# jl6017/AutoURDF

Measured on AMD Instinct MI355X. Metric: registered frames/sec (N=4096 pts, K=20 clusters), higher is better.
Workload: dtype f32

## Files before the change

### autourdf_amd/_lib.py

```python
import ctypes
import os

import torch

_HERE = os.path.dirname(os.path.abspath(__file__))
_VARIANT = os.environ.get("CREG_LIB_VARIANT", "")
LIB_PATH = os.path.join(_HERE, "libcreg" + ("_" + _VARIANT if _VARIANT else "") + ".so")

vp, i64, i32, f32, f64, sz = (ctypes.c_void_p, ctypes.c_int64, ctypes.c_int32, ctypes.c_float,
                              ctypes.c_double, ctypes.c_size_t)


class TrainShape(ctypes.Structure):
    _fields_ = [("rot", i32), ("k", i32), ("hidden", i32), ("epochs", i32), ("n_pred", i64),
                ("n_tgt", i64), ("use_graph", i32), ("batch", i32), ("graph_branches", i32), ("nn_search", i32)]


class TrainArgs(ctypes.Structure):
    _fields_ = [("m", vp), ("y", vp), ("local_pts", vp), ("seg_offsets", vp),
                ("params", ctypes.POINTER(vp)), ("lr", f32), ("sched_factor", f32),
                ("sched_patience", i32), ("stop", i32), ("best_m", vp), ("best_pred", vp),
                ("loss_hist", vp), ("lr_hist", vp), ("result", vp), ("y_unchanged", i32), ("reserved_", i32)]


# ... 56 lines not shown
    "creg_depth_points_f64": (ctypes.c_int, [vp, vp, i32, f64, f64, i32, i32, vp, sz, vp, i64, vp]),
    "creg_segment_plane_workspace_bytes": (sz, [i64, i32, i32]),
    "creg_segment_plane_f64": (ctypes.c_int, [vp, i64, vp, i32, vp, i32, i32, f64, vp, vp, vp, vp, vp, vp, vp, sz, vp]),
    "creg_mesh_collide_workspace_bytes": (sz, [i64, i32, i64, i64]),
    "creg_mesh_collide_f64": (ctypes.c_int, [vp, vp, i64, vp, i32, i64, vp, i64, vp, vp, vp, vp, sz, vp]),
    "creg_urdf_fk_f64": (ctypes.c_int, [vp, vp, vp, vp, vp, i32, i32, i32, vp, i32, vp, vp, vp, vp]),
    "creg_coord_dist_map_workspace_bytes": (sz, [i32, i32]),
    "creg_coord_dist_map_f64": (ctypes.c_int, [vp, i32, i32, f64, i32, vp, vp, vp, sz, vp]),
    "creg_pose_coords_f64": (ctypes.c_int, [vp, i64, vp, vp]),
    "creg_link_sweep_f64": (ctypes.c_int, [vp, i32, i32, i32, vp, vp, vp, vp, vp, vp]),
    "creg_coord_mst_f64": (ctypes.c_int, [vp, i32, i32, vp, vp, vp]),
    "creg_joint_axes_samples": (ctypes.c_int, [i32, i32, i32]),
    "creg_joint_axes_f64": (ctypes.c_int, [vp, i32, i32, i32, vp, vp, i32, vp, i32, i32, i32, i32, vp, vp, vp, vp, vp, vp, vp,
                                           vp, vp, vp, vp]),
    "creg_link_clouds_f64": (ctypes.c_int, [vp, vp, i32, i32, vp, vp, i32, i32, vp, vp, i64, vp, i64, i64, vp, vp, vp, vp,
                                            vp]),
    "creg_statistical_outlier_f64": (ctypes.c_int, [vp, i64, vp, i32, i32, f64, vp, vp, vp, vp]),
    "creg_voxel_bounds_f64": (ctypes.c_int, [vp, i64, vp, i32, vp, f64, vp, vp, vp, vp]),
    "creg_voxel_layout": (ctypes.c_int, [vp, vp, i32, vp]),
    "creg_voxel_fill_f64": (ctypes.c_int, [vp, i64, vp, i32, vp, f64, vp, vp, vp, i64, vp, vp]),
    "creg_mc_workspace_bytes": (sz, [i64]),
    "creg_mc_count_u8": (ctypes.c_int, [vp, vp, vp, i32, i64, vp, vp, vp, sz, vp]),
    "creg_mc_emit_i32": (ctypes.c_int, [vp, vp, i32, i64, vp, i64, i64, vp, vp, vp, sz, vp]),
    "creg_mesh_finish_workspace_bytes": (sz, [i64]),
    "creg_mesh_finish_f64": (ctypes.c_int, [vp, i64, vp, i64, vp, vp, i32, vp, f64, i32, vp, vp, vp, sz, vp]),
    "creg_train_workspace_bytes": (sz, [ctypes.POINTER(TrainShape)]),
    "creg_train_plan_create": (ctypes.c_int, [ctypes.POINTER(TrainShape), vp, sz, ctypes.POINTER(vp)]),
    "creg_train_plan_run": (ctypes.c_int, [vp, ctypes.POINTER(TrainArgs), vp]),
    "creg_train_plan_run_batch": (ctypes.c_int, [vp, ctypes.POINTER(TrainArgs), i32, vp]),
    "creg_train_plan_resume": (ctypes.c_int, [vp, ctypes.POINTER(TrainArgs), ctypes.POINTER(TrainState), i32, ctypes.POINTER(vp), ctypes.POINTER(vp), vp, vp]),
    "creg_train_plan_probe": (ctypes.c_int, [vp, ctypes.POINTER(TrainArgs), vp, vp, vp, vp, vp]),
    "creg_train_plan_profile": (ctypes.c_int, [vp, ctypes.POINTER(TrainArgs), i32, ctypes.POINTER(f32), vp]),
    "creg_train_plan_info": (ctypes.c_int, [vp, vp]),
    "creg_train_plan_destroy": (ctypes.c_int, [vp]),
}

_lib = None


def load(check_device: bool = True) -> ctypes.CDLL:
    global _lib
    if _lib is None:
        if not os.path.exists(LIB_PATH):
            raise RuntimeError(
                f"{LIB_PATH} is missing: build it with `python -m autourdf_amd.build` "
                "(hipcc --offload-arch=gfx950). autourdf_amd has no CPU fallback.")
        hip = os.path.join(os.path.dirname(torch.__file__), "lib", "libamdhip64.so")
        if os.path.exists(hip):
            ctypes.CDLL(hip, mode=ctypes.RTLD_GLOBAL)
        L = ctypes.CDLL(LIB_PATH)
        for name, (res, args) in SIGNATURES.items():
            fn = getattr(L, name)
            fn.restype, fn.argtypes = res, args
        _lib = L
    if check_device:
        rc = _lib.creg_device_check()
        if rc != 0:
            raise RuntimeError("libcreg needs an MI355X (gfx950): " + _lib.creg_last_error().decode())
    return _lib


def check(rc: int, what: str = "libcreg call"):
    if rc != 0:
        raise RuntimeError(f"{what} failed ({rc}): {_lib.creg_last_error().decode()}")


# ... 8 lines not shown
```

### autourdf_amd/csrc/train_engine.hip

```cpp
#include <cfloat>
#include <chrono>
#include <cmath>
#include <cstdlib>
#include <cstring>
#include <type_traits>
#include <vector>
#include "creg_common.h"
#include "nn_l1.h"

namespace creg {

struct Dims {
    int rot, K, KP, IN, H, HA, HB, H2, OA, OB, NP, NT, epochs;
    float slope;
    int oW1, ob1, oW2, ob2, oW3A, ob3A, oW3B, ob3B, NPAR;
    int nbx, nby;
    int nyb;
    int npb;
    int ppl;
    int nbt, nbp;
    int rows;
};

constexpr int PS_MAXB = 512;
// ... 1 lines not shown
struct Hyper {
    float lr, factor;
    int patience, stop;
};

struct TrainState {
    double lr, sched_best;
    int sched_bad, count, stopped, step;
    float min_loss;
    int epochs_run, best_epoch;
    float step_size, bc2_sqrt;
    float last_loss;
    float next_bc2s;
    double next_bc1;
};

struct Ws {
    float *P, *P1, *AM, *AV;
    float *pose_in, *enc, *x1[2], *h2[2], *head_save, *m2, *gm2;
    float4 *pts4, *y4, *pred4, *ys4, *psl4, *ps4;
    float *ybox, *pbox;
    int* sb;
    int* sgn_x;
    int4* cnt4;
    float *lossp_x, *lossp_y;
    float *g_out, *g_h2;
    TrainState* state;
    double* bc1;
    float* bc2s;
    float *best_m, *best_pred, *loss_hist, *lr_hist, *result;
    int* off;
    Hyper* hyper;
    unsigned long long* ysum;
};

static_assert(sizeof(Ws) % sizeof(char*) == 0, "Ws must hold pointers only");
__host__ __device__ __forceinline__ Ws ws_shift(Ws W, size_t bytes) {
    char** p = reinterpret_cast<char**>(&W);
#pragma unroll
    for (size_t i = 0; i < sizeof(Ws) / sizeof(char*); ++i) p[i] += bytes;
    return W;
}

constexpr int ROT_Q = 0, ROT_DQ = 1, ROT_6D = 2, ROT_RPY = 3;
constexpr int POSE_IN = 12;
__device__ __forceinline__ float act_f(float v, float slope) { return v > 0.f ? v : v * slope; }
__device__ __forceinline__ float act_grad(float post, float slope) { return post > 0.f ? 1.f : slope; }

__device__ __forceinline__ int seg_of(const int* __restrict__ off, int k, int n) {
    int lo = 0, hi = k;
    while (hi - lo > 1) { const int mid = (lo + hi) >> 1; if (off[mid] <= n) lo = mid; else hi = mid; }
    return lo;
}

constexpr int PREP_MAXB = 64;
struct PrepBatch { const float* m[PREP_MAXB]; const float* y[PREP_MAXB]; const float* pts[PREP_MAXB]; Hyper hy[PREP_MAXB]; };
__global__ __launch_bounds__(256) void k_prep(Dims D, Ws W0, size_t bstride, PrepBatch pb) {
    const Ws W = ws_shift(W0, blockIdx.z * bstride);
    const Hyper hy = pb.hy[blockIdx.z];
    const float* __restrict__ m = pb.m[blockIdx.z];
    const float* __restrict__ y = pb.y[blockIdx.z];
    const float* __restrict__ pts = pb.pts[blockIdx.z];
    const int t = blockIdx.x * 256 + threadIdx.x;
    const int stride = gridDim.x * 256;
    for (int n = t; n < D.NP; n += stride) {
        const int c = seg_of(W.off, D.K, n);
// ... 71 lines not shown
}

typedef float f32x4 __attribute__((ext_vector_type(4)));
constexpr int L2_THREADS = 512;
constexpr int L2_RB = 32;
template <int NC>
__device__ __forceinline__ void l2_body(const Dims& D, const Ws& W, int par, int blk) {
    constexpr int KW = 8 * NC, NS = KW / 4;
    constexpr bool V4 = KW % 16 == 0;
    constexpr int NL = V4 ? NS / 4 : NS;
    __shared__ __attribute__((aligned(16))) float red[(L2_THREADS / 64) * L2_RB * 16];
    const float* Pc = par ? W.P1 : W.P;
    const float* x1cur = par ? W.x1[1] : W.x1[0];
    float* h2out = par ? W.h2[1] : W.h2[0];
    const int tid = threadIdx.x, lane = tid & 63, wv = tid >> 6, lj = lane & 15, kk = lane >> 4;
    const int u0 = blk * 16, H = D.H;
    auto load_t = [&](const float* rowp, float* dst) {
        const float* p = rowp + wv * KW + (V4 ? 4 * kk : kk);
#pragma unroll
        for (int q = 0; q < NL; ++q) {
            if constexpr (V4) { const float4 v = *(const float4*)(p + 16 * q); dst[4 * q] = v.x; dst[4 * q + 1] = v.y; dst[4 * q + 2] = v.z; dst[4 * q + 3] = v.w; }
            else dst[q] = p[4 * q];
        }
    };
    float bw[NS], a0[NS], a1[NS];
    load_t(Pc + D.oW2 + (size_t)(u0 + lj) * H, bw);
    load_t(x1cur + (size_t)min(lj, D.K - 1) * H, a0);
    const bool two0 = D.K > 16;
    if (two0) load_t(x1cur + (size_t)min(16 + lj, D.K - 1) * H, a1);
    const float bias = Pc[D.ob2 + u0 + (tid & 15)];
    __builtin_amdgcn_sched_barrier(0);
    const int stopped = W.state[par].stopped;
    __builtin_amdgcn_sched_barrier(0);
    for (int r0 = 0; r0 < D.K; r0 += L2_RB) {
        const int nr = min(L2_RB, D.K - r0);
        const bool two = nr > 16;
        if (r0) {
            load_t(x1cur + (size_t)min(r0 + lj, D.K - 1) * H, a0);
            if (two) load_t(x1cur + (size_t)min(r0 + 16 + lj, D.K - 1) * H, a1);
        }
        f32x4 acc0 = {0.f, 0.f, 0.f, 0.f}, acc1 = {0.f, 0.f, 0.f, 0.f};
        if (two) {
#pragma unroll
            for (int s = 0; s < NS; ++s) {
                acc0 = __builtin_amdgcn_mfma_f32_16x16x4f32(a0[s], bw[s], acc0, 0, 0, 0);
                acc1 = __builtin_amdgcn_mfma_f32_16x16x4f32(a1[s], bw[s], acc1, 0, 0, 0);
            }
        } else {
#pragma unroll
            for (int s = 0; s < NS; ++s) acc0 = __builtin_amdgcn_mfma_f32_16x16x4f32(a0[s], bw[s], acc0, 0, 0, 0);
        }
        if (r0) __syncthreads();
        {
            float* o = red + (wv * L2_RB + 4 * kk) * 16 + lj;
#pragma unroll
            for (int v = 0; v < 4; ++v) { o[v * 16] = acc0[v]; if (two) o[(16 + v) * 16] = acc1[v]; }
        }
        __syncthreads();
        if (stopped) return;
        if (tid < nr * 16) {
            float sum = red[tid];
#pragma unroll
            for (int w2 = 1; w2 < L2_THREADS / 64; ++w2) sum += red[w2 * L2_RB * 16 + tid];
            h2out[(size_t)(r0 + (tid >> 4)) * D.H2 + u0 + (tid & 15)] = act_f(sum + bias, D.slope);
        }
    }
}
template <int NC>
__global__ __launch_bounds__(L2_THREADS) void k_l2(Dims D, Ws W0, int par, size_t bstride) {
    asm volatile("" :: "s"(W0.P), "s"(W0.P1), "s"(W0.x1[0]), "s"(W0.x1[1]), "s"(W0.h2[0]), "s"(W0.h2[1]), "s"(W0.state), "s"(D.K), "s"(D.H),
                 "s"(D.H2), "s"(D.oW2), "s"(D.ob2), "s"(D.slope), "s"(par), "s"(bstride));
    const Ws W = ws_shift(W0, blockIdx.z * bstride);
    l2_body<NC>(D, W, par, blockIdx.x);
}

template <int NC, bool X = false>
__global__ __launch_bounds__(512) void k_head(Dims D, Ws W0, int par, size_t bstride) {
    asm volatile("" :: "s"(W0.P), "s"(W0.P1), "s"(W0.h2[0]), "s"(W0.h2[1]), "s"(W0.pose_in), "s"(W0.head_save), "s"(W0.m2), "s"(W0.pts4), "s"(W0.pred4),
                 "s"(W0.psl4), "s"(W0.ps4), "s"(W0.pbox), "s"(W0.sb), "s"(W0.cnt4), "s"(W0.state), "s"(W0.off), "s"(D.rot), "s"(D.K), "s"(D.H2), "s"(D.HA),
                 "s"(D.HB), "s"(D.OA), "s"(D.OB), "s"(D.NP), "s"(D.npb), "s"(D.ppl), "s"(D.nbp), "s"(D.oW3A), "s"(D.ob3A), "s"(D.oW3B), "s"(D.ob3B), "s"(par),
                 "s"(bstride));
    const Ws W = ws_shift(W0, blockIdx.z * bstride);
    const float* h2cur = par ? W.h2[1] : W.h2[0];
    const float* Pc = par ? W.P1 : W.P;
    __shared__ float outs[12];
    __shared__ float m2s[12];
    const int r = blockIdx.x, lane = threadIdx.x & 63, wave = threadIdx.x >> 6;
    const int NO = D.OA + D.OB;
    const int o = min(wave, (X ? 8 : NO) - 1);
    const float *w, *a; int n;
    if (o < D.OA) { w = Pc + D.oW3A + (size_t)o * D.HA; a = h2cur + (size_t)r * D.H2; n = D.HA; }
    else { w = Pc + D.oW3B + (size_t)(o - D.OA) * D.HB; a = h2cur + (size_t)r * D.H2 + D.HA; n = D.HB; }
    float wv[NC], av[NC];
#pragma unroll
    for (int c = 0; c < NC; ++c) { const int i = min(c * 64 + lane, n - 1); wv[c] = w[i]; av[c] = a[i]; }
    const float bias = o < D.OA ? Pc[D.ob3A + o] : Pc[D.ob3B + o - D.OA];
    float wv9[NC], av9[NC], bias9 = 0.f;
    if constexpr (X) {
        const float* w9 = Pc + D.oW3B + (size_t)(8 - D.OA) * D.HB;
        const float* a9 = h2cur + (size_t)r * D.H2 + D.HA;
#pragma unroll
        for (int c = 0; c < NC; ++c) { const int i = min(c * 64 + lane, D.HB - 1); wv9[c] = w9[i]; av9[c] = a9[i]; }
        bias9 = Pc[D.ob3B + 8 - D.OA];
// ... 594 lines not shown
constexpr int B2_WAVES = B2_THREADS / 64;
constexpr int B2_CB = 16;
constexpr int B2_RB = 32;
__host__ __device__ inline int b2_smem_floats(int K, int IN, int H2) {
    return B2_WAVES * B2_RB * B2_CB + K * IN + 2 * K * B2_CB + H2 * B2_CB;
}
__device__ __forceinline__ float row_sum16(float v) {
    CREG_DPP_STEP(v, 0xB1, 0xF);
    CREG_DPP_STEP(v, 0x4E, 0xF);
    CREG_DPP_STEP(v, 0x141, 0xF);
    CREG_DPP_STEP(v, 0x140, 0xF);
    return v;
}

template <int KW, bool X>
__device__ __forceinline__ void bwd2_role(const Dims& D, const Ws& W, int epoch, int blk, float* sh, unsigned long long bd_entry) {
    constexpr int NS = KW / 4;
    constexpr bool V4 = KW % 16 == 0;
    constexpr int NA = V4 ? NS / 4 : NS;
    float* red = sh;
    float* encs = red + B2_WAVES * B2_RB * B2_CB;
    float* gxs = encs + D.K * D.IN;
    float* xt = gxs + D.K * B2_CB;
    float* w2s = xt + D.K * B2_CB;
    const int tid = threadIdx.x, lane = tid & 63, wv = tid >> 6, lj = lane & 15, kk = lane >> 4;
    __builtin_amdgcn_s_waitcnt(0x0F70);
    const int c0 = blk * B2_CB, par = epoch & 1;
    const float* x1cur = par ? W.x1[1] : W.x1[0];
    float* x1next = par ? W.x1[0] : W.x1[1];
    const float* Pc = par ? W.P1 : W.P;
    float* Pn = par ? W.P : W.P1;
    BD_T0
    {
        const float* src = Pc + D.oW2 + (size_t)(wv * KW + (lane >> 2)) * D.H + c0 + 4 * (lane & 3);
        float* dst = w2s + wv * KW * B2_CB;
#pragma unroll
        for (int i = 0; i < KW; i += 16)
            if (i + (lane >> 2) < KW)
                __builtin_amdgcn_global_load_lds((const __attribute__((address_space(1))) void*)(src + (size_t)i * D.H),
                                                 (__attribute__((address_space(3))) void*)(dst + i * B2_CB), 16, 0, 0);
    }
    const float* gbase = W.g_h2 + wv * KW + (V4 ? 4 * kk : kk);
    auto load_a = [&](int row, float* dst) {
        const float* g = gbase + (size_t)min(row, D.K - 1) * D.H2;
#pragma unroll
        for (int q = 0; q < NA; ++q) {
            if constexpr (V4) { const float4 v = *(const float4*)(g + 16 * q); dst[4 * q] = v.x; dst[4 * q + 1] = v.y; dst[4 * q + 2] = v.z; dst[4 * q + 3] = v.w; }
            else dst[q] = g[4 * q];
        }
    };
    float a0[NS], a1[NS];
    const bool two0 = D.K > 16;
    load_a(lj, a0);
    if (two0) load_a(16 + lj, a1);
    const int half = tid >> 8, t2 = tid & 255, row = t2 >> 4, i4 = t2 & 15, hu = c0 + row;
    const bool ain = 4 * i4 < D.IN;
    const int ei = min(4 * i4, D.IN - 4);
    const size_t wi = (size_t)D.oW1 + (size_t)hu * D.IN + ei;
    float4 pw = *(const float4*)(Pc + wi), pm = *(const float4*)(W.AM + wi), pv = *(const float4*)(W.AV + wi);
    const bool ain2 = X && 64 + 4 * i4 < D.IN;
    const int ei2 = min(64 + 4 * i4, D.IN - 4);
    const size_t wi2 = (size_t)D.oW1 + (size_t)hu * D.IN + ei2;
    float4 pw2, pm2, pv2;
    if constexpr (X) { pw2 = *(const float4*)(Pc + wi2); pm2 = *(const float4*)(W.AM + wi2); pv2 = *(const float4*)(W.AV + wi2); }
    float pb = Pc[D.ob1 + hu], mb = W.AM[D.ob1 + hu], vb = W.AV[D.ob1 + hu];
    float xv0 = x1cur[(size_t)min(tid >> 4, D.K - 1) * D.H + c0 + (tid & 15)];
    {
        const int n = D.K * D.IN / 4;
        constexpr int NPC = 8;
#pragma unroll
        for (int c = 0; c < NPC; ++c) {
            const int i = c * B2_THREADS + tid;
// ... 181 lines not shown
        mfma_ops();
    }
    BD_T
    if (S.stopped) return;
#pragma unroll
    for (int v = 0; v < DW_TILES; ++v) {
        float4 nw;
        nw.x = adam_value(pw[v].x, pm[v].x, pv[v].x, acc[0][v], S.step_size, S.bc2_sqrt);
        nw.y = adam_value(pw[v].y, pm[v].y, pv[v].y, acc[1][v], S.step_size, S.bc2_sqrt);
        nw.z = adam_value(pw[v].z, pm[v].z, pv[v].z, acc[2][v], S.step_size, S.bc2_sqrt);
        nw.w = adam_value(pw[v].w, pm[v].w, pv[v].w, acc[3][v], S.step_size, S.bc2_sqrt);
        if (vl[v]) { const int e = po / 4 + 16 * v; st4_wt(Pn, e, nw); st4_wt(W.AM, e, pm[v]); st4_wt(W.AV, e, pv[v]); }
    }
    if (wv == 0) {
        float sum = gb;
        sum += __shfl_xor(gb, 16, 64);
        sum += __shfl_xor(sum, 32, 64);
        pb = adam_value(pb, mb, vb, sum, S.step_size, S.bc2_sqrt);
        if (q == 0 && ulive) { Pn[ob + unit] = pb; W.AM[ob + unit] = mb; W.AV[ob + unit] = vb; }
    }
    BD_TEND(1, epoch);
}

template <int NC, int KW, bool X = false>
__global__ __launch_bounds__(BD_THREADS, 4) void k_bd(Dims D, Ws W0, int epoch, size_t bstride, int nz) {
    extern __shared__ __attribute__((aligned(16))) char smem[];
#ifdef CREG_BD_STAMPS
    const unsigned long long bd_entry = wall_clock64();
#else
    const unsigned long long bd_entry = 0;
#endif
#ifndef CREG_BD_NO_TOUCH
    asm volatile("" :: "s"(W0.P), "s"(W0.P1), "s"(W0.AM), "s"(W0.AV), "s"(W0.enc), "s"(W0.x1[0]), "s"(W0.x1[1]), "s"(W0.h2[0]), "s"(W0.h2[1]),
                 "s"(W0.g_out), "s"(W0.g_h2), "s"(W0.state), "s"(D.K), "s"(D.KP), "s"(D.IN), "s"(D.H), "s"(D.H2), "s"(D.HA), "s"(D.HB), "s"(D.OA),
                 "s"(D.OB), "s"(D.oW1), "s"(D.ob1), "s"(D.oW2), "s"(D.ob2), "s"(D.oW3A), "s"(D.ob3A), "s"(D.oW3B), "s"(D.ob3B), "s"(D.NPAR),
                 "s"(D.slope), "s"(epoch), "s"(bstride), "s"(nz));
#endif
    const int nB = D.H / B2_CB, nD = dw_blocks(D);
    int i = blockIdx.x;
    const bool roleB = i < nB * nz;
    if (!roleB) i -= nB * nz;
    const int n = roleB ? nB : nD, z = i / n, blk = i - z * n;
    const Ws W = ws_shift(W0, (size_t)z * bstride);
#ifdef CREG_BD_ONLY
    if ((CREG_BD_ONLY == 1) != roleB) return;
#endif
    if (roleB) bwd2_role<KW, X>(D, W, epoch, blk, (float*)smem, bd_entry);
    else dw_role(D, W, epoch, blk, bd_entry);
}

__global__ __launch_bounds__(256) void k_params_home(Dims D, Ws W0, size_t bstride, int sidx, int step0) {
    const Ws W = ws_shift(W0, blockIdx.z * bstride);
    if (((W.state[sidx].step - step0) & 1) == 0) return;
    for (int i = blockIdx.x * 256 + threadIdx.x; i < D.NPAR; i += gridDim.x * 256) W.P[i] = W.P1[i];
}

struct ResumeState { double lr, sched_best; int step, epochs_run, sched_bad, count, best_epoch, stopped; float min_loss; };
__global__ void k_set_state(Dims D, Ws W, ResumeState rs) {
    if (threadIdx.x || blockIdx.x) return;
    TrainState s = W.state[0];
    s.lr = rs.lr; s.sched_best = rs.sched_best; s.sched_bad = rs.sched_bad; s.count = rs.count; s.stopped = rs.stopped; s.step = rs.step;
    s.min_loss = rs.min_loss; s.epochs_run = rs.epochs_run; s.best_epoch = rs.best_epoch;
    s.next_bc1 = W.bc1[min(rs.step + 1, D.epochs)]; s.next_bc2s = W.bc2s[min(rs.step + 1, D.epochs)];
    W.state[0] = s; W.state[1] = s;
    W.result[0] = s.min_loss; W.result[1] = (float)s.epochs_run; W.result[2] = (float)s.lr; W.result[3] = (float)s.best_epoch;
}
__global__ void k_get_state(Ws W, int sidx, double* out) {
    if (threadIdx.x || blockIdx.x) return;
    const TrainState s = W.state[sidx];
    out[0] = s.step; out[1] = s.epochs_run; out[2] = s.lr; out[3] = s.sched_best; out[4] = s.sched_bad; out[5] = s.count;
    out[6] = (double)s.min_loss; out[7] = s.best_epoch; out[8] = s.stopped; out[9] = (double)s.last_loss; out[10] = 0.0; out[11] = 0.0;
}

struct Plan {
    creg_train_shape shape;
    Dims D;
    Ws W;
    char* base;
    size_t bytes;
    hipGraphExec_t gexec;
    bool graph_ready;
    int graph_epochs;
    int B;
    size_t bstride;
    int smem_bd;
    int branches;
    bool chain_streams;
    hipStream_t cst[8];
    hipGraphExec_t cexec[8];
    hipEvent_t cfork, cjoin[8];
    hipStream_t cal_stream;
    bool cal_done;
    int probe_us;
    bool target_blocks_valid;
};

struct Slice { Ws W; int nz; };
static Slice slice_of(const Plan* P, int first, int count) { return Slice{ws_shift(P->W, (size_t)first * P->bstride), count}; }
static Slice chain_slice(const Plan* P, int gi) {
    const int q = P->B / P->branches, r = P->B % P->branches;
    return slice_of(P, gi * q + (gi < r ? gi : r), q + (gi < r ? 1 : 0));
}

static bool make_dims(const creg_train_shape* s, Dims* D) {
// ... 29 lines not shown
    const int nt = (D->nyb + 63) / 64, np = (D->npb + 63) / 64;
    D->nbt = nt <= 1 ? 1 : (nt <= 2 ? 2 : 4);
    D->nbp = np <= 2 ? 2 : (np <= 3 ? 3 : (np <= 4 ? 4 : (np <= 5 ? 5 : (np <= 6 ? 6 : 8))));
    if (D->rows) { D->nbx = 4 * D->npb; D->nby = 4 * D->nyb; }
    return true;
}

static size_t carve(const Dims& D, char* base, Ws* W) {
    size_t o = 0;
    auto take = [&](size_t bytes) -> char* { char* r = base ? base + o : nullptr; o = align_up(o + bytes, 256); return r; };
    const size_t f = sizeof(float);
    Ws w;
    w.P = (float*)take(f * D.NPAR); w.P1 = (float*)take(f * D.NPAR); w.AM = (float*)take(f * D.NPAR); w.AV = (float*)take(f * D.NPAR);
    w.pose_in = (float*)take(f * POSE_IN * D.K); w.enc = (float*)take(f * D.K * D.IN);
    w.x1[0] = (float*)take(f * D.KP * D.H); w.x1[1] = (float*)take(f * D.KP * D.H);
    w.h2[0] = (float*)take(f * D.KP * D.H2); w.h2[1] = (float*)take(f * D.KP * D.H2); w.head_save = (float*)take(f * 16 * D.K);
    w.m2 = (float*)take(f * 16 * D.K); w.gm2 = (float*)take(f * 16 * D.K);
    w.pts4 = (float4*)take(sizeof(float4) * D.NP); w.y4 = (float4*)take(sizeof(float4) * D.NT);
    w.pred4 = (float4*)take(sizeof(float4) * D.NP);
    const size_t bs = 64 * (size_t)D.ppl;
    w.ys4 = (float4*)take(sizeof(float4) * bs * (D.nyb ? D.nyb : 1)); w.ybox = (float*)take(f * 6 * 64 * D.nbt);
    w.psl4 = (float4*)take(sizeof(float4) * bs * (D.npb ? D.npb : 1)); w.ps4 = (float4*)take(sizeof(float4) * bs * (D.npb ? D.npb : 1));
    w.pbox = (float*)take(f * 6 * 64 * D.nbp); w.sb = (int*)take(sizeof(int) * (D.K + 1));
    w.sgn_x = (int*)take(sizeof(int) * D.NP);
    w.cnt4 = (int4*)take(sizeof(int4) * D.NP);
    w.lossp_x = (float*)take(f * D.nbx); w.lossp_y = (float*)take(f * D.nby);
    w.g_out = (float*)take(f * 16 * D.KP); w.g_h2 = (float*)take(f * D.KP * D.H2);
    w.state = (TrainState*)take(sizeof(TrainState) * 2);
    w.bc1 = (double*)take(sizeof(double) * (D.epochs + 1)); w.bc2s = (float*)take(f * (D.epochs + 1));
    w.best_m = (float*)take(f * 16 * D.K); w.best_pred = (float*)take(f * 3 * D.NP);
    w.loss_hist = (float*)take(f * D.epochs); w.lr_hist = (float*)take(f * D.epochs); w.result = (float*)take(f * 4);
    w.off = (int*)take(sizeof(int) * (D.K + 1)); w.hyper = (Hyper*)take(sizeof(Hyper));
    w.ysum = (unsigned long long*)take(sizeof(unsigned long long) * 4);
    if (W) *W = w;
    return o;
}

template <typename F>
static void by_nc(int H, F f) {
    switch (H / 64) {
        case 1: f(std::integral_constant<int, 1>{}); break;
        case 2: f(std::integral_constant<int, 2>{}); break;
        case 4: f(std::integral_constant<int, 4>{}); break;
        default: f(std::integral_constant<int, 8>{}); break;
    }
}
static void launch_l2(const Plan* P, const Slice& S, int par, hipStream_t s) {
    const Dims& D = P->D;
    by_nc(D.H, [&](auto nc) {
        hipLaunchKernelGGL((k_l2<decltype(nc)::value>), dim3(D.H2 / 16, 1, S.nz), dim3(L2_THREADS), 0, s, D, S.W, par, P->bstride); });
}
static void launch_head(const Plan* P, const Slice& S, int par, hipStream_t s) {
    const Dims& D = P->D;
    by_nc(D.H, [&](auto nc) {
        if (D.OA + D.OB > 8) hipLaunchKernelGGL((k_head<decltype(nc)::value, true>), dim3(D.K, 1, S.nz), dim3(512), 0, s, D, S.W, par, P->bstride);
        else hipLaunchKernelGGL((k_head<decltype(nc)::value>), dim3(D.K, 1, S.nz), dim3(512), 0, s, D, S.W, par, P->bstride);
    });
}
template <typename F>
static void by_bd(const Dims& D, F f) {
    by_nc(D.H, [&](auto nc) {
        constexpr int NC = decltype(nc)::value;
        if (D.IN > 64) f(k_bd<NC, 12 * NC, true>);
        else if (D.HA) f(k_bd<NC, 12 * NC>);
        else f(k_bd<NC, 8 * NC>);
    });
// ... 510 lines not shown
    for (int e = 0; e < n_epochs; ++e)
        for (int k = 0; k < NKERN; ++k) {
            float ms = 0.f;
            CREG_HIP(hipEventElapsedTime(&ms, ev[(NKERN + 1) * e + k], ev[(NKERN + 1) * e + k + 1]));
            acc[k] += ms;
        }
    us_out[0] = 0.f;
    for (int k = 0; k < NKERN; ++k) us_out[1 + k] = (float)(acc[k] * 1000.0 / n_epochs);
    const int REP = 200;
    const Dims& D = P->D; const Ws& W = P->W;
    CREG_HIP(hipEventRecord(ev[0], s));
    for (int i = 0; i < REP; ++i)
        launch_nn(D, W, P->bstride, S.nz, s);
    CREG_HIP(hipEventRecord(ev[1], s));
    CREG_HIP(hipStreamSynchronize(s));
    float ms = 0.f;
    CREG_HIP(hipEventElapsedTime(&ms, ev[0], ev[1]));
    us_out[6] = ms * 1000.f / REP;
    us_out[7] = (float)S.nz;
    auto b2b = [&](auto launch, float* out) -> int {
        CREG_HIP(hipEventRecord(ev[0], s));
        for (int i = 0; i < REP; ++i) launch(i);
        CREG_HIP(hipEventRecord(ev[1], s));
        CREG_HIP(hipStreamSynchronize(s));
        CREG_HIP(hipEventElapsedTime(&ms, ev[0], ev[1]));
        *out = ms * 1000.f / REP;
        return CREG_OK;
    };
#ifdef CREG_BD_STAMPS
    {   BdStamps* z = new BdStamps; memset(z, 0, sizeof(*z)); memset(z->first, 0xff, sizeof(z->first)); memset(z->startB, 0xff, sizeof(z->startB));
        memset(z->startD, 0xff, sizeof(z->startD)); z->armed = 1;
        CREG_HIP(hipMemcpyToSymbol(HIP_SYMBOL(g_bd_st), z, sizeof(*z))); delete z; }
#endif
    if (int rc2 = b2b([&](int i) { launch_bd(P, S, i, s); }, us_out + 8)) return rc2;
#ifdef CREG_BD_STAMPS
    { const int zero = 0; CREG_HIP(hipMemcpyToSymbol(HIP_SYMBOL(g_bd_st), &zero, sizeof(int), offsetof(BdStamps, armed))); }
#endif
    if (int rc2 = b2b([&](int i) { launch_l2(P, S, i & 1, s); }, us_out + 9)) return rc2;
    if (int rc2 = b2b([&](int i) { launch_head(P, S, i & 1, s); }, us_out + 10)) return rc2;
    if (int rc2 = b2b([&](int i) { hipLaunchKernelGGL(k_gradc, dim3(D.K, 1, S.nz), dim3(256), 0, s, D, W, i, D.nbx, D.nby, P->bstride); }, us_out + 11)) return rc2;
    CREG_LAUNCH_CHECK();
    return CREG_OK;
}

#ifdef CREG_BD_STAMPS
extern "C" int creg_debug_bd_stamps(double* out) {
    BdStamps* z = new BdStamps;
    if (hipMemcpyFromSymbol(z, HIP_SYMBOL(g_bd_st), sizeof(*z)) != hipSuccess) { delete z; return CREG_EHIP; }
    for (int i = 0; i < 24; ++i) out[i] = 0.0;
    int n = 0;
    for (int sl = 0; sl < 256; ++sl) {
        if (z->first[sl] == ~0ull || !z->endB[sl] || !z->endD[sl]) continue;
        ++n;
        const double f = (double)z->first[sl];
        out[0] += ((double)(z->endB[sl] > z->endD[sl] ? z->endB[sl] : z->endD[sl]) - f) / 100.0;
        out[1] += ((double)z->startB[sl] - f) / 100.0; out[2] += ((double)z->endB[sl] - f) / 100.0;
        out[3] += ((double)z->startD[sl] - f) / 100.0; out[4] += ((double)z->endD[sl] - f) / 100.0;
    }
    for (int i = 0; i < 5; ++i) out[i] /= n ? n : 1;
    out[5] = n ? (double)z->blocks[0] / n : 0; out[6] = n ? (double)z->blocks[1] / n : 0; out[7] = n;
    for (int r = 0; r < 2; ++r)
        for (int k = 0; k < 8; ++k) out[8 + 8 * r + k] = z->blocks[r] ? (double)z->phase[r][k] / (double)z->blocks[r] / 100.0 : 0.0;
    delete z;
    return CREG_OK;
}
#endif

#ifdef CREG_NN_STATS
extern "C" int creg_debug_nn_stats(unsigned long long* out8, int reset) {
    CREG_HIP(hipMemcpyFromSymbol(out8, HIP_SYMBOL(creg::g_nn_stats), sizeof(unsigned long long) * 8));
    if (reset) { unsigned long long z[8] = {0}; CREG_HIP(hipMemcpyToSymbol(HIP_SYMBOL(creg::g_nn_stats), z, sizeof(z))); }
    return CREG_OK;
}
#endif

#ifdef CREG_NN_WAVE_STAMPS
extern "C" long long creg_debug_nn_waves(unsigned long long* out, long long cap, int reset) {
    static unsigned n[creg::NN_WAVE_SHARDS * 32];
    if (hipMemcpyFromSymbol(n, HIP_SYMBOL(creg::g_nn_wave_n), sizeof(n)) != hipSuccess) return -1;
    long long total = 0;
    if (out && cap > 0) {
        std::vector<creg::NnWaveRec> h((size_t)creg::NN_WAVE_CAP);
        if (hipMemcpyFromSymbol(h.data(), HIP_SYMBOL(creg::g_nn_wave), sizeof(creg::NnWaveRec) * (size_t)creg::NN_WAVE_CAP) != hipSuccess) return -1;
        for (unsigned sh = 0; sh < creg::NN_WAVE_SHARDS; ++sh) {
            const unsigned m = n[32 * sh] < creg::NN_WAVE_PER ? n[32 * sh] : creg::NN_WAVE_PER;
            for (unsigned i = 0; i < m && total < cap; ++i, ++total) {
                const creg::NnWaveRec& r = h[(size_t)sh * creg::NN_WAVE_PER + i];
                unsigned long long* o = out + 8 * total;
                o[0] = r.t0; o[1] = r.t1; o[2] = r.t2; o[3] = r.t3; o[4] = (unsigned long long)r.visits; o[5] = (unsigned long long)r.cands;
                o[6] = (unsigned long long)r.dir; o[7] = (unsigned long long)r.blk;
            }
        }
    } else for (unsigned sh = 0; sh < creg::NN_WAVE_SHARDS; ++sh) total += n[32 * sh];
    if (reset) { static const unsigned z[creg::NN_WAVE_SHARDS * 32] = {}; if (hipMemcpyToSymbol(HIP_SYMBOL(creg::g_nn_wave_n), z, sizeof(z)) != hipSuccess) return -1; }
    return total;
}
#endif


extern "C" int creg_train_plan_info(const creg_train_plan* plan, creg_train_plan_info_t* info) {
    CREG_REQUIRE(plan && info, "creg_train_plan_info: null pointer");
    const Plan* P = (const Plan*)plan;
    info->pruned_target_search = P->D.rows ? 2 : (P->D.nyb > 0);
    info->pruned_predicted_search = P->D.npb > 0;
    info->graph_branches = P->branches;
    info->batch = P->B;
    info->epochs_per_graph = P->shape.use_graph ? P->graph_epochs : 0;
    info->nn_points_per_lane = P->D.ppl;
    info->nn_boxes_target = P->D.nbt;
    info->nn_boxes_predicted = P->D.nbp;
    info->chain_probe_us = P->probe_us;
    return CREG_OK;
}

extern "C" int creg_train_plan_destroy(creg_train_plan* plan) {
    Plan* P = (Plan*)plan;
    if (!P) return CREG_OK;
    if (P->gexec) (void)hipGraphExecDestroy(P->gexec);
    for (int i = 0; i < 8; ++i) {
        if (P->cst[i]) (void)hipStreamSynchronize(P->cst[i]);
        if (P->cexec[i]) (void)hipGraphExecDestroy(P->cexec[i]);
        if (P->cjoin[i]) (void)hipEventDestroy(P->cjoin[i]);
        if (P->cst[i]) (void)hipStreamDestroy(P->cst[i]);
    }
    if (P->cfork) (void)hipEventDestroy(P->cfork);
    delete P;
    return CREG_OK;
}
```

### autourdf_amd/ops.py

```python
import ctypes

import numpy as np

import torch

from . import _lib


def _stream():
    return ctypes.c_void_p(torch.cuda.current_stream().cuda_stream)


def _need(t: torch.Tensor, dtype, name: str) -> torch.Tensor:
    if not isinstance(t, torch.Tensor) or not t.is_cuda:
        raise RuntimeError(f"{name} must be a CUDA tensor on the MI355X (autourdf_amd has no CPU path)")
    if t.dtype != dtype:
        raise TypeError(f"{name} must be {dtype}, got {t.dtype}")
    return t.contiguous()


def _p(t):
    return ctypes.c_void_p(t.data_ptr()) if t is not None else None


# ... 994 lines not shown
        a = self._args(m, y, pts, offsets, params, float(state.get("lr", 2e-4)), factor, patience, stop, o)
        st = _lib.TrainState()
        arr_a = (ctypes.c_void_p * n)(*[q.data_ptr() for q in ea])
        arr_s = (ctypes.c_void_p * n)(*[q.data_ptr() for q in es])
        st.exp_avg, st.exp_avg_sq = ctypes.cast(arr_a, ctypes.POINTER(ctypes.c_void_p)), ctypes.cast(arr_s, ctypes.POINTER(ctypes.c_void_p))
        st.lr, st.sched_best = float(state.get("lr", 2e-4)), float(state.get("sched_best", float("inf")))
        st.step, st.epochs_run = int(state.get("step", 0)), int(state.get("epochs_run", state.get("step", 0)))
        st.sched_bad, st.count, st.best_epoch, st.stopped = int(state.get("sched_bad", 0)), int(state.get("count", 0)), best_epoch, int(state.get("stopped", 0))
        st.min_loss = float(state.get("min_loss", 1000.0))
        ea2, es2 = [torch.empty_like(q) for q in ea], [torch.empty_like(q) for q in es]
        out_a = (ctypes.c_void_p * n)(*[q.data_ptr() for q in ea2])
        out_s = (ctypes.c_void_p * n)(*[q.data_ptr() for q in es2])
        sc = torch.empty(12, dtype=torch.float64, device=self.device)
        _lib.check(self.L.creg_train_plan_resume(self.plan, ctypes.byref(a), ctypes.byref(st), int(n_epochs),
                                                 ctypes.cast(out_a, ctypes.POINTER(ctypes.c_void_p)), ctypes.cast(out_s, ctypes.POINTER(ctypes.c_void_p)),
                                                 _p(sc), _stream()), "creg_train_plan_resume")
        h = sc.cpu().tolist()
        after = {"exp_avg": ea2, "exp_avg_sq": es2, "last_loss": h[9]}
        for i, k in enumerate(self.STATE_FIELDS):
            after[k] = h[i] if k in ("lr", "sched_best", "min_loss") else int(h[i])
        return o[0], o[1], o[4], o[2], o[3], after

    def probe(self, m, y, pts, offsets, params):
        dev = self.device
        m2 = torch.empty(self.k, 4, 4, dtype=torch.float32, device=dev)
        pred = torch.empty(self.n_pred, 3, dtype=torch.float32, device=dev)
        loss = torch.empty(1, dtype=torch.float32, device=dev)
        gm = torch.empty(self.k, 4, 4, dtype=torch.float32, device=dev)
        a = self._args(m, y, pts, offsets, params, 2e-4, 0.7, 5, 200, (None, None, None, None, None))
        _lib.check(self.L.creg_train_plan_probe(self.plan, ctypes.byref(a), _p(m2), _p(pred), _p(loss), _p(gm),
                                                _stream()), "creg_train_plan_probe")
        return m2, pred, loss, gm

    KERNELS = ("_", "head", "nn_l1", "gradc", "bd", "l2")

    def profile(self, m, y, pts, offsets, params, n_epochs=50):
        out = (ctypes.c_float * 16)()
        a = self._args(m, y, pts, offsets, params, 2e-4, 0.7, 5, 200, (None, None, None, None, None))
        _lib.check(self.L.creg_train_plan_profile(self.plan, ctypes.byref(a), n_epochs, out, _stream()),
                   "creg_train_plan_profile")
        d = dict(zip(self.KERNELS, [float(v) for v in out]))
        d.pop("_")
        d["nn_l1_back_to_back"] = float(out[6])
        d["nn_l1_problems_per_launch"] = int(out[7])
        d["bd_back_to_back"] = float(out[8])
        d["l2_back_to_back"] = float(out[9])
        d["head_back_to_back"] = float(out[10])
        d["gradc_back_to_back"] = float(out[11])
        return d
```

### include/creg.h

```cpp
#ifndef CREG_H
#define CREG_H

#include <stddef.h>
#include <stdint.h>

#ifdef __cplusplus
extern "C" {
#endif

typedef void* creg_stream_t;

enum creg_status {
    CREG_OK = 0,
    CREG_EINVAL = -1,
    CREG_EHIP = -2,
    CREG_ENOTCONVERGED = -3,
    CREG_EARCH = -4
};

int creg_version(void);
const char* creg_last_error(void);
int creg_device_check(void);

int creg_nn_l1_bidir_f32(const float* x, int64_t nx, const float* y, int64_t ny,
// ... 210 lines not shown
} creg_train_plan_info_t;

size_t creg_train_workspace_bytes(const creg_train_shape* shape);
int creg_train_plan_create(const creg_train_shape* shape, void* workspace, size_t workspace_bytes,
                           creg_train_plan** plan);
int creg_train_plan_run(creg_train_plan* plan, const creg_train_args* args, creg_stream_t stream);
int creg_train_plan_run_batch(creg_train_plan* plan, const creg_train_args* args, int32_t n, creg_stream_t stream);
int creg_train_plan_info(const creg_train_plan* plan, creg_train_plan_info_t* info);
int creg_train_plan_destroy(creg_train_plan* plan);

typedef struct creg_train_state {
    float* const* exp_avg;
    float* const* exp_avg_sq;
    double lr;
    double sched_best;
    int32_t step;
    int32_t epochs_run;
    int32_t sched_bad;
    int32_t count;
    int32_t best_epoch;
    int32_t stopped;
    float min_loss;
    int32_t reserved_;
} creg_train_state;
int creg_train_plan_resume(creg_train_plan* plan, const creg_train_args* args, const creg_train_state* from, int32_t n_epochs,
                           float* const* exp_avg_out, float* const* exp_avg_sq_out, double* state_out, creg_stream_t stream);

int creg_train_plan_probe(creg_train_plan* plan, const creg_train_args* args, float* m2,
                          float* pred, float* loss, float* grad_m2, creg_stream_t stream);

int creg_train_plan_profile(creg_train_plan* plan, const creg_train_args* args, int32_t n_epochs,
                            float* us_out, creg_stream_t stream);

#ifdef __cplusplus
}
#endif
#endif
```

Before: 164.7.

## Write a tiled W2 shadow copy in l2 for contiguous backward-kernel loads

The layer-2 forward kernel now writes its already-loaded W2 weight fragments into a tiled, transposed shadow buffer laid out in 16-column blocks. The backward (bd) kernel reads W2 from that shadow, so its global-to-LDS loads become contiguous instead of strided by the hidden dimension. This costs extra global stores in l2 and a new workspace buffer, and relies on l2 running before bd with the current weights. A mismatch-check kernel and API are added to validate that the shadow matches the parameters.

Result: slower. 162.4 (-1.4%).

```diff
diff --git a/autourdf_amd/_lib.py b/autourdf_amd/_lib.py
--- a/autourdf_amd/_lib.py
+++ b/autourdf_amd/_lib.py
@@ -112,6 +112,7 @@
     "creg_train_plan_probe": (ctypes.c_int, [vp, ctypes.POINTER(TrainArgs), vp, vp, vp, vp, vp]),
     "creg_train_plan_profile": (ctypes.c_int, [vp, ctypes.POINTER(TrainArgs), i32, ctypes.POINTER(f32), vp]),
     "creg_train_plan_info": (ctypes.c_int, [vp, vp]),
+    "creg_train_plan_w2_shadow_mismatches": (ctypes.c_int, [vp, i32, vp, vp]),
     "creg_train_plan_destroy": (ctypes.c_int, [vp]),
 }
 
diff --git a/autourdf_amd/csrc/train_engine.hip b/autourdf_amd/csrc/train_engine.hip
--- a/autourdf_amd/csrc/train_engine.hip
+++ b/autourdf_amd/csrc/train_engine.hip
@@ -57,6 +57,7 @@
     int* off;
     Hyper* hyper;
     unsigned long long* ysum;
+    float* w2t;
 };
 
 static_assert(sizeof(Ws) % sizeof(char*) == 0, "Ws must hold pointers only");
@@ -194,6 +195,19 @@
     __builtin_amdgcn_sched_barrier(0);
     const int stopped = W.state[par].stopped;
     __builtin_amdgcn_sched_barrier(0);
+    if (!stopped) {
+        if constexpr (V4) {
+#pragma unroll
+            for (int q = 0; q < NL; ++q)
+                st4_wt(W.w2t, ((wv * (KW / 16) + q) * D.H2 + u0 + lj) * 16 + 4 * kk, make_float4(bw[4 * q], bw[4 * q + 1], bw[4 * q + 2], bw[4 * q + 3]));
+        } else {
+#pragma unroll
+            for (int q = 0; q < NL; ++q) {
+                const int c = wv * KW + 4 * q + kk;
+                W.w2t[((size_t)(c >> 4) * D.H2 + u0 + lj) * 16 + (c & 15)] = bw[q];
+            }
+        }
+    }
     for (int r0 = 0; r0 < D.K; r0 += L2_RB) {
         const int nr = min(L2_RB, D.K - r0);
         const bool two = nr > 16;
@@ -230,7 +244,7 @@
 }
 template <int NC>
 __global__ __launch_bounds__(L2_THREADS) void k_l2(Dims D, Ws W0, int par, size_t bstride) {
-    asm volatile("" :: "s"(W0.P), "s"(W0.P1), "s"(W0.x1[0]), "s"(W0.x1[1]), "s"(W0.h2[0]), "s"(W0.h2[1]), "s"(W0.state), "s"(D.K), "s"(D.H),
+    asm volatile("" :: "s"(W0.P), "s"(W0.P1), "s"(W0.x1[0]), "s"(W0.x1[1]), "s"(W0.h2[0]), "s"(W0.h2[1]), "s"(W0.state), "s"(W0.w2t), "s"(D.K), "s"(D.H),
                  "s"(D.H2), "s"(D.oW2), "s"(D.ob2), "s"(D.slope), "s"(par), "s"(bstride));
     const Ws W = ws_shift(W0, blockIdx.z * bstride);
     l2_body<NC>(D, W, par, blockIdx.x);
@@ -891,12 +905,12 @@
     float* Pn = par ? W.P : W.P1;
     BD_T0
     {
-        const float* src = Pc + D.oW2 + (size_t)(wv * KW + (lane >> 2)) * D.H + c0 + 4 * (lane & 3);
+        const float* src = W.w2t + ((size_t)blk * D.H2 + wv * KW + (lane >> 2)) * B2_CB + 4 * (lane & 3);
         float* dst = w2s + wv * KW * B2_CB;
 #pragma unroll
         for (int i = 0; i < KW; i += 16)
             if (i + (lane >> 2) < KW)
-                __builtin_amdgcn_global_load_lds((const __attribute__((address_space(1))) void*)(src + (size_t)i * D.H),
+                __builtin_amdgcn_global_load_lds((const __attribute__((address_space(1))) void*)(src + i * B2_CB),
                                                  (__attribute__((address_space(3))) void*)(dst + i * B2_CB), 16, 0, 0);
     }
     const float* gbase = W.g_h2 + wv * KW + (V4 ? 4 * kk : kk);
@@ -1144,7 +1158,7 @@
 #endif
 #ifndef CREG_BD_NO_TOUCH
     asm volatile("" :: "s"(W0.P), "s"(W0.P1), "s"(W0.AM), "s"(W0.AV), "s"(W0.enc), "s"(W0.x1[0]), "s"(W0.x1[1]), "s"(W0.h2[0]), "s"(W0.h2[1]),
-                 "s"(W0.g_out), "s"(W0.g_h2), "s"(W0.state), "s"(D.K), "s"(D.KP), "s"(D.IN), "s"(D.H), "s"(D.H2), "s"(D.HA), "s"(D.HB), "s"(D.OA),
+                 "s"(W0.g_out), "s"(W0.g_h2), "s"(W0.state), "s"(W0.w2t), "s"(D.K), "s"(D.KP), "s"(D.IN), "s"(D.H), "s"(D.H2), "s"(D.HA), "s"(D.HB), "s"(D.OA),
                  "s"(D.OB), "s"(D.oW1), "s"(D.ob1), "s"(D.oW2), "s"(D.ob2), "s"(D.oW3A), "s"(D.ob3A), "s"(D.oW3B), "s"(D.ob3B), "s"(D.NPAR),
                  "s"(D.slope), "s"(epoch), "s"(bstride), "s"(nz));
 #endif
@@ -1182,6 +1196,15 @@
     const TrainState s = W.state[sidx];
     out[0] = s.step; out[1] = s.epochs_run; out[2] = s.lr; out[3] = s.sched_best; out[4] = s.sched_bad; out[5] = s.count;
     out[6] = (double)s.min_loss; out[7] = s.best_epoch; out[8] = s.stopped; out[9] = (double)s.last_loss; out[10] = 0.0; out[11] = 0.0;
+}
+
+__global__ __launch_bounds__(256) void k_w2_shadow_diff(Dims D, Ws W, int* count) {
+    int bad = 0;
+    for (int i = blockIdx.x * 256 + threadIdx.x; i < D.H2 * D.H; i += gridDim.x * 256) {
+        const int o = i / D.H, c = i - o * D.H;
+        bad += __float_as_int(W.P[D.oW2 + i]) != __float_as_int(W.w2t[((size_t)(c >> 4) * D.H2 + o) * 16 + (c & 15)]);
+    }
+    if (bad) atomicAdd(count, bad);
 }
 
 struct Plan {
@@ -1277,6 +1300,7 @@
     w.loss_hist = (float*)take(f * D.epochs); w.lr_hist = (float*)take(f * D.epochs); w.result = (float*)take(f * 4);
     w.off = (int*)take(sizeof(int) * (D.K + 1)); w.hyper = (Hyper*)take(sizeof(Hyper));
     w.ysum = (unsigned long long*)take(sizeof(unsigned long long) * 4);
+    w.w2t = (float*)take(f * D.H * D.H2);
     if (W) *W = w;
     return o;
 }
@@ -1853,7 +1877,11 @@
         memset(z->startD, 0xff, sizeof(z->startD)); z->armed = 1;
         CREG_HIP(hipMemcpyToSymbol(HIP_SYMBOL(g_bd_st), z, sizeof(*z))); delete z; }
 #endif
+#ifdef CREG_BD_STAMPS
+    if (int rc2 = b2b([&](int i) { launch_bd(P, S, i, s); launch_l2(P, S, (i + 1) & 1, s); }, us_out + 8)) return rc2;
+#else
     if (int rc2 = b2b([&](int i) { launch_bd(P, S, i, s); }, us_out + 8)) return rc2;
+#endif
 #ifdef CREG_BD_STAMPS
     { const int zero = 0; CREG_HIP(hipMemcpyToSymbol(HIP_SYMBOL(g_bd_st), &zero, sizeof(int), offsetof(BdStamps, armed))); }
 #endif
@@ -1919,6 +1947,17 @@
 #endif
 
 
+extern "C" int creg_train_plan_w2_shadow_mismatches(creg_train_plan* plan, int32_t slot, int32_t* count_dev, creg_stream_t stream) {
+    Plan* P = (Plan*)plan;
+    CREG_REQUIRE(P && count_dev, "creg_train_plan_w2_shadow_mismatches: null pointer");
+    CREG_REQUIRE(slot >= 0 && slot < P->B, "creg_train_plan_w2_shadow_mismatches: slot %d of a plan for %d problems", slot, P->B);
+    hipStream_t s = (hipStream_t)stream;
+    CREG_HIP(hipMemsetAsync(count_dev, 0, sizeof(int32_t), s));
+    hipLaunchKernelGGL(k_w2_shadow_diff, dim3(cdiv(P->D.H2 * P->D.H, 256)), dim3(256), 0, s, P->D, slice_of(P, slot, 1).W, count_dev);
+    CREG_LAUNCH_CHECK();
+    return CREG_OK;
+}
+
 extern "C" int creg_train_plan_info(const creg_train_plan* plan, creg_train_plan_info_t* info) {
     CREG_REQUIRE(plan && info, "creg_train_plan_info: null pointer");
     const Plan* P = (const Plan*)plan;
diff --git a/autourdf_amd/ops.py b/autourdf_amd/ops.py
--- a/autourdf_amd/ops.py
+++ b/autourdf_amd/ops.py
@@ -1050,6 +1050,12 @@
                                                 _stream()), "creg_train_plan_probe")
         return m2, pred, loss, gm
 
+    def w2_shadow_mismatches(self, slot: int = 0) -> int:
+        count = torch.empty(1, dtype=torch.int32, device=self.device)
+        _lib.check(self.L.creg_train_plan_w2_shadow_mismatches(self.plan, int(slot), _p(count), _stream()),
+                   "creg_train_plan_w2_shadow_mismatches")
+        return int(count.item())
+
     KERNELS = ("_", "head", "nn_l1", "gradc", "bd", "l2")
 
     def profile(self, m, y, pts, offsets, params, n_epochs=50):
diff --git a/include/creg.h b/include/creg.h
--- a/include/creg.h
+++ b/include/creg.h
@@ -266,6 +266,8 @@
 int creg_train_plan_profile(creg_train_plan* plan, const creg_train_args* args, int32_t n_epochs,
                             float* us_out, creg_stream_t stream);
 
+int creg_train_plan_w2_shadow_mismatches(creg_train_plan* plan, int32_t slot, int32_t* count_dev, creg_stream_t stream);
+
 #ifdef __cplusplus
 }
 #endif
```
